# Deam0on/deepEMIA

Measured on AMD Instinct MI355X. Metric: EM tiles/s (2048x2048, R101-FPN), higher is better.
Workload: dtype f16x2

## Files before the change

### deepemia_amd/csrc/conv_p32.hip

```cpp
#include <utility>
#include "common.h"
#ifndef P32_ABLATE
#define P32_ABLATE 0
#endif

#ifndef P32_HEAD_DIRECT
#define P32_HEAD_DIRECT 1
#endif
#ifndef P32_SINGLE
#define P32_SINGLE 0
#endif
#ifndef P32_DEV_TILES
#define P32_DEV_TILES 0
#endif
#ifndef P32_ST_AUX
#define P32_ST_AUX 0
#endif
#ifndef P32_RES_AUX
#define P32_RES_AUX 0
#endif
#ifndef P32_A_NT
#define P32_A_NT 0
#endif
#ifndef P32_FRAG_PIPE
#define P32_FRAG_PIPE 0
#endif

namespace {

struct ConvQ {
    const void* in;
    const float* in_meta;
    const void* w;
    const float* scale;
    const float* bias;
    const void* res;
    const float* res_meta;
    void* out;
    float* out_meta;
    float wbound, bbound;
    int N, H, W, Cin, Ho, Wo, Cout, CoutPad, KH, KW, stride, pad;
    int act, res_mode, out_f32, out_ld;
    int M, HoWo, ntn, nwg, ksteps, taps;
    int kloop;
    unsigned in_bytes, w_bytes;
    unsigned out_bytes, res_bytes;
    const float* head_w;
    const float* head_b;
    float* head_out;
    int head_n, head_ld, head_act;
    int groups, group_rows, row0;
    int no_hk;
    int zero_low;
    int stagger_ticks;
    int resident;
};

typedef __attribute__((address_space(3))) void lds_void;

template <int OFF, int WAIT>
__device__ __forceinline__ void ds_read2_b128(f16x8& a, f16x8& b, unsigned addr_a, unsigned addr_b) {
    if constexpr (WAIT >= 0)
        asm volatile("ds_read_b128 %0, %2 offset:%4\n\tds_read_b128 %1, %3 offset:%4\n\ts_waitcnt lgkmcnt(%5)"
                     : "=&v"(a), "=&v"(b) : "v"(addr_a), "v"(addr_b), "n"(OFF), "n"(WAIT) : "memory");
    else
        asm volatile("ds_read_b128 %0, %2 offset:%4\n\tds_read_b128 %1, %3 offset:%4"
                     : "=&v"(a), "=&v"(b) : "v"(addr_a), "v"(addr_b), "n"(OFF) : "memory");
}

template <int... Is, class F>
__device__ __forceinline__ void static_for_impl(std::integer_sequence<int, Is...>, F&& f) { (f(std::integral_constant<int, Is>{}), ...); }
template <int N, class F>
__device__ __forceinline__ void static_for(F&& f) { static_for_impl(std::make_integer_sequence<int, N>{}, static_cast<F&&>(f)); }
typedef int i32x4 __attribute__((ext_vector_type(4)));

__device__ __forceinline__ void dma16(const i32x4 rsrc, unsigned lds_addr, unsigned voff, unsigned soff) {
    unsigned keep;
    asm volatile("s_mov_b32 %0, m0\n\ts_mov_b32 m0, %1\n\ts_nop 0\n\tbuffer_load_dwordx4 %2, %3, %4 offen lds\n\ts_mov_b32 m0, %0"
                 : "=&s"(keep) : "s"(lds_addr), "v"(voff), "s"(rsrc), "s"(soff) : "memory");
}
__device__ __forceinline__ void dma16_nt(const i32x4 rsrc, unsigned lds_addr, unsigned voff, unsigned soff) {
    unsigned keep;
    asm volatile("s_mov_b32 %0, m0\n\ts_mov_b32 m0, %1\n\ts_nop 0\n\tbuffer_load_dwordx4 %2, %3, %4 offen nt lds\n\ts_mov_b32 m0, %0"
                 : "=&s"(keep) : "s"(lds_addr), "v"(voff), "s"(rsrc), "s"(soff) : "memory");
}
__device__ __forceinline__ i32x4 make_rsrc(const void* base, unsigned bytes) {
    const unsigned long long a = reinterpret_cast<unsigned long long>(base);
    i32x4 r;
    r[0] = __builtin_amdgcn_readfirstlane((int)(unsigned)a);
    r[1] = __builtin_amdgcn_readfirstlane((int)((unsigned)(a >> 32) & 0xffffu));
    r[2] = __builtin_amdgcn_readfirstlane((int)bytes);
    r[3] = 0x00020000;
    return r;
}

__device__ __forceinline__ float apply_act_q(float v, int act) {
    if (act == DEMIA_ACT_RELU) return v > 0.f ? v : 0.f;
    if (act == DEMIA_ACT_SIGMOID) return 1.0f / (1.0f + expf(-v));
    return v;
}

__device__ __forceinline__ float plane_scale(float bound) {
    if (!(bound > 0.f) || !(bound < 3.0e38f)) return 1.f;
    int e = 14 - ilogbf(bound);
    e = e < -100 ? -100 : (e > 100 ? 100 : e);
    return ldexpf(1.f, e);
}

template <int TN, int EF>
__device__ __forceinline__ void write_acc32(const f32x16 (&row)[TN], float* e, int lane) {
#pragma unroll
    for (int j = 0; j < TN; ++j)
#pragma unroll
        for (int r = 0; r < 16; ++r)
            e[((r & 3) + 8 * (r >> 2) + 4 * (lane >> 5)) * EF + j * 32 + (lane & 31)] = row[j][r];
}
template <int TN, int EF>
__device__ __forceinline__ void write_acc16(const f32x4 (&r0)[2 * TN], const f32x4 (&r1)[2 * TN], float* e, int lane) {
#pragma unroll
    for (int j = 0; j < 2 * TN; ++j)
#pragma unroll
        for (int r = 0; r < 4; ++r) {
            e[(4 * (lane >> 4) + r) * EF + j * 16 + (lane & 15)] = r0[j][r];
            e[(16 + 4 * (lane >> 4) + r) * EF + j * 16 + (lane & 15)] = r1[j][r];
        }
}

__device__ __forceinline__ float uniform(float v) { return __int_as_float(__builtin_amdgcn_readfirstlane(__float_as_int(v))); }

struct GroupScales {
    int g0, b1, b2;
    float post0, post1, post2, resi0, resi1, resi2, sout0, sout1, sout2;
};

__device__ __forceinline__ void load_group_scale(const ConvQ& p, int gi, bool planes_out, float& post, float& resi, float& sout) {
    gi = min(gi, p.groups - 1);
    const float amax_in = p.in_meta[2 * gi], s_in = p.in_meta[2 * gi + 1];
    float amax_res = 0.f, s_res = 1.f;
    if (p.res_mode != DEMIA_RES_NONE) { amax_res = p.res_meta[2 * gi]; s_res = p.res_meta[2 * gi + 1]; }
    post = uniform(1.0f / s_in);
    resi = uniform(p.res_mode != DEMIA_RES_NONE ? 1.0f / s_res : 0.f);
    sout = uniform(planes_out ? plane_scale(amax_in * p.wbound + p.bbound + amax_res) : 1.f);
}

__device__ __forceinline__ GroupScales load_group_scales(const ConvQ& p, int m0, bool planes_out) {
    GroupScales gs;
    gs.g0 = (m0 + p.row0) / p.group_rows;
    gs.b1 = (gs.g0 + 1) * p.group_rows - p.row0;
    gs.b2 = gs.b1 + p.group_rows;
    load_group_scale(p, gs.g0, planes_out, gs.post0, gs.resi0, gs.sout0);
    load_group_scale(p, gs.g0 + 1, planes_out, gs.post1, gs.resi1, gs.sout1);
    load_group_scale(p, gs.g0 + 2, planes_out, gs.post2, gs.resi2, gs.sout2);
    return gs;
}

template <int WM, int WN, int TM, int TN, bool HEAD, typename WriteRow>
__device__ __forceinline__ void p32_epilogue(const ConvQ& p, const GroupScales& gs, char* smem, WriteRow&& write_tile_row, int wm, int wn, int m0, int n0) {
    constexpr int BN = WN * TN * 32;
    const int tid = threadIdx.x, lane = tid & 63;
    constexpr int EROW = BN * 4 + 16;
    constexpr int GPR = BN / 8, RSTEP = 512 / GPR, ITEMS = WM * 32 / RSTEP;
    static_assert(512 % GPR == 0 && (WM * 32) % RSTEP == 0, "epilogue split");
    constexpr int BM_ = WM * TM * 32;
    static_assert(!HEAD || BN == 256, "the fused head needs a 256-wide tile");
    const bool planes_out = !HEAD && !p.out_f32;
    const int g0 = __builtin_amdgcn_readfirstlane(gs.g0), b1 = __builtin_amdgcn_readfirstlane(gs.b1), b2 = __builtin_amdgcn_readfirstlane(gs.b2);
    const float post0 = uniform(gs.post0), post1 = uniform(gs.post1), post2 = uniform(gs.post2);
    const float resi0 = uniform(gs.resi0), resi1 = uniform(gs.resi1), resi2 = uniform(gs.resi2);
    const float sout0 = uniform(gs.sout0), sout1 = uniform(gs.sout1), sout2 = uniform(gs.sout2);
    if (planes_out && n0 == 0 && tid == 0) {
#pragma unroll
        for (int d = 0; d < 3; ++d) {
            const int first = d == 0 ? g0 * p.group_rows - p.row0 : (d == 1 ? b1 : b2);
            if (g0 + d < p.groups && first >= m0 && first < m0 + BM_ && first < p.M)
                p.out_meta[2 * (g0 + d) + 1] = d == 0 ? sout0 : (d == 1 ? sout1 : sout2);
        }
    }
    const int g = tid % GPR, r_first = tid / GPR;
    const int co = n0 + g * 8;
    float sc[8], bs[8];
#pragma unroll
    for (int q = 0; q < 8; ++q) {
        const bool ok = (co + q) < p.Cout;
        sc[q] = (p.scale && ok) ? p.scale[co + q] : 1.0f;
        bs[q] = (p.bias && ok) ? p.bias[co + q] : 0.0f;
    }
    float vmax3[3] = {0.f, 0.f, 0.f};
    constexpr int HMAX = 4;
    float hw[HMAX][8];
    constexpr bool head_on = HEAD;
    if (head_on) {
#pragma unroll
        for (int j = 0; j < HMAX; ++j)
#pragma unroll
            for (int q = 0; q < 8; ++q) hw[j][q] = j < p.head_n ? p.head_w[j * 256 + g * 8 + q] : 0.f;
    }
    const int tile_n_ = n0 / BN;
    const bool res_on = p.res_mode != DEMIA_RES_NONE, sigmoid_on = p.act == DEMIA_ACT_SIGMOID;
    const float act_lo = p.act == DEMIA_ACT_RELU ? 0.f : -INFINITY;
    const char* resb = reinterpret_cast<const char*>(p.res) + 128;
    char* outb = reinterpret_cast<char*>(p.out) + 128;
    const long cbytes = (long)p.Cout * 4;
    const int gofs = (co >> 5) * 128 + ((co & 31) >> 3) * 16;
    auto row_of = [&](int i, int k) { const int lr = r_first + k * RSTEP; return m0 + (lr >> 5) * (TM * 32) + i * 32 + (lr & 31); };
    auto res_pix = [&](int m) -> long {
        if (p.res_mode == DEMIA_RES_SAME) return m;
        const int n = m / p.HoWo;
        const int rem = m - n * p.HoWo;
// ... 194 lines not shown
    load_res(0);
#pragma unroll
    for (int i = 0; i < TM; ++i) {
        asm volatile("" ::: "memory");
        __builtin_amdgcn_wave_barrier();
        write_tile_row(i, reinterpret_cast<float*>(wsm));
        asm volatile("" ::: "memory");
        __builtin_amdgcn_wave_barrier();
        f16x8 ch[ITEMS], cl[ITEMS];
#pragma unroll
        for (int k = 0; k < ITEMS; ++k) {
            ch[k] = __builtin_bit_cast(f16x8, from_below(rh[k], rl[k]));
            cl[k] = __builtin_bit_cast(f16x8, from_above(rl[k], rh[k]));
        }
        if (i + 1 < TM) load_res(i + 1);
#pragma unroll
        for (int k = 0; k < ITEMS; ++k) {
            const int lr = r_first + k * RPI;
            const int m = row_of(i, k);
            const float4 x0 = *reinterpret_cast<const float4*>(wsm + lr * (LDW * 4) + (line * 4 + cj) * 32);
            const float4 x1 = *reinterpret_cast<const float4*>(wsm + lr * (LDW * 4) + (line * 4 + cj) * 32 + 16);
            typedef float f32x2 __attribute__((ext_vector_type(2)));
            f32x2 v2[4] = {{x0.x, x0.y}, {x0.z, x0.w}, {x1.x, x1.y}, {x1.z, x1.w}};
            const int gd = (m >= b1) + (m >= b2);
            const float post = gd == 0 ? post0 : (gd == 1 ? post1 : post2);
            const float res_inv = gd == 0 ? resi0 : (gd == 1 ? resi1 : resi2);
            const float s_out = gd == 0 ? sout0 : (gd == 1 ? sout1 : sout2);
            float v[8];
#pragma unroll
            for (int q = 0; q < 4; ++q) {
                const f32x2 scq = {sc[2 * q], sc[2 * q + 1]}, bsq = {bs[2 * q], bs[2 * q + 1]};
                const f32x2 t = (v2[q] * post) * scq + bsq;
                v[2 * q] = t.x;
                v[2 * q + 1] = t.y;
            }
#pragma unroll
            for (int q = 0; q < 8; ++q) {
                v[q] = fmaf((float)cl[k][q], res_inv, fmaf((float)ch[k][q], res_inv, v[q]));
                v[q] = fmaxf(v[q], act_lo);
            }
            if (sigmoid_on && !(P32_ABLATE & 256)) {
#pragma unroll
                for (int q = 0; q < 8; ++q) v[q] = 1.0f / (1.0f + expf(-v[q]));
            }
            f16x8 h, l;
            float vm = 0.f;
#pragma unroll
            for (int q = 0; q < 8; q += 2) {
                vm = fmaxf(vm, fmaxf(fabsf(v[q]), fabsf(v[q + 1])));
                const f32x2 y = f32x2{v[q], v[q + 1]} * s_out;
                h[q] = (_Float16)y.x;
                h[q + 1] = (_Float16)y.y;
                l[q] = (_Float16)fmaf(-(float)h[q], 1.0f, y.x);
                l[q + 1] = (_Float16)fmaf(-(float)h[q + 1], 1.0f, y.y);
            }
            if (single) l = f16x8{0, 0, 0, 0, 0, 0, 0, 0};
            vm = m < p.M ? vm : 0.f;
            vmax0 = fmaxf(vmax0, gd == 0 ? vm : 0.f);
            vmax1 = fmaxf(vmax1, gd == 1 ? vm : 0.f);
            vmax2 = fmaxf(vmax2, gd == 2 ? vm : 0.f);
            const u32x4 hu = __builtin_bit_cast(u32x4, h), lu = __builtin_bit_cast(u32x4, l);
            const u32x4 d0 = from_below(hu, lu);
            const u32x4 d1 = from_above(lu, hu);
            const unsigned off = (unsigned)(m - rs) * cbytes + lofs;
            if (P32_ABLATE & 64) {
                asm volatile("" :: "v"(d0), "v"(d1), "v"(off));
            } else {
                __builtin_amdgcn_raw_buffer_store_b128(d0, rs_out, off, 0, P32_ST_AUX);
                __builtin_amdgcn_raw_buffer_store_b128(d1, rs_out, off + cbytes, 0, P32_ST_AUX);
            }
            hook();
        }
    }
#pragma unroll
    for (int d = 0; d < 3; ++d) {
        if (d > 0 && (d == 1 ? b1 : b2) >= m0 + BM_) break;
        if (g0 + d >= p.groups) break;
        float vmax = d == 0 ? vmax0 : (d == 1 ? vmax1 : vmax2);
#pragma unroll
        for (int o = 32; o > 0; o >>= 1) vmax = fmaxf(vmax, __shfl_xor(vmax, o));
        float* slot = p.out_meta + 2 * (g0 + d);
        if (lane == 0 && vmax > *reinterpret_cast<volatile const float*>(slot))
            atomicMax(reinterpret_cast<unsigned int*>(slot), __float_as_uint(vmax));
    }
}

template <int WM, int WN, int TM, int TN, int HN>
__device__ __forceinline__ void p32_epilogue_head_direct(const ConvQ& p, const GroupScales& gs, char* smem, const f32x4 (&acc16)[2 * TM][2 * TN],
                                                         int wm, int wn, int m0, int n0) {
    constexpr int BM = WM * TM * 32, BN = WN * TN * 32;
    static_assert(BN == 256, "the fused head needs a 256-wide tile");
    const int tid = threadIdx.x, lane = tid & 63, c16 = lane & 15, rq = lane >> 4;
    const int b1 = __builtin_amdgcn_readfirstlane(gs.b1), b2 = __builtin_amdgcn_readfirstlane(gs.b2);
    const float post0 = uniform(gs.post0), post1 = uniform(gs.post1), post2 = uniform(gs.post2);
    float sc[2 * TN], bs[2 * TN], hw[HN][2 * TN];
#pragma unroll
    for (int jn = 0; jn < 2 * TN; ++jn) {
        const int cl = wn * TN * 32 + jn * 16 + c16;
        sc[jn] = p.scale ? p.scale[n0 + cl] : 1.0f;
        bs[jn] = p.bias ? p.bias[n0 + cl] : 0.0f;
#pragma unroll
        for (int j = 0; j < HN; ++j) hw[j][jn] = j < p.head_n ? p.head_w[j * 256 + cl] : 0.f;
    }
    const float act_lo = p.act == DEMIA_ACT_RELU ? 0.f : -INFINITY;
    float* part = reinterpret_cast<float*>(smem);
#pragma unroll
    for (int i = 0; i < 2 * TM; ++i) {
#pragma unroll
        for (int r = 0; r < 4; ++r) {
            const int row = wm * TM * 32 + i * 16 + rq * 4 + r;
            const int m = m0 + row;
            const int gd = (m >= b1) + (m >= b2);
            const float post = gd == 0 ? post0 : (gd == 1 ? post1 : post2);
            float a[HN];
#pragma unroll
            for (int j = 0; j < HN; ++j) a[j] = 0.f;
#pragma unroll
            for (int jn = 0; jn < 2 * TN; ++jn) {
                const float v = fmaxf((acc16[i][jn][r] * post) * sc[jn] + bs[jn], act_lo);
#pragma unroll
                for (int j = 0; j < HN; ++j) a[j] = fmaf(v, hw[j][jn], a[j]);
            }
#pragma unroll
            for (int j = 0; j < HN; ++j) {
                a[j] += __int_as_float(__builtin_amdgcn_update_dpp(0, __float_as_int(a[j]), 0x128, 0xf, 0xf, false));
                a[j] += __int_as_float(__builtin_amdgcn_update_dpp(0, __float_as_int(a[j]), 0x124, 0xf, 0xf, false));
                a[j] += __int_as_float(__builtin_amdgcn_update_dpp(0, __float_as_int(a[j]), 0x122, 0xf, 0xf, false));
                a[j] += __int_as_float(__builtin_amdgcn_update_dpp(0, __float_as_int(a[j]), 0x121, 0xf, 0xf, false));
            }
            if (c16 == 0) {
#pragma unroll
                for (int j = 0; j < HN; ++j) part[((long)wn * BM + row) * HN + j] = a[j];
            }
        }
    }
    __syncthreads();
    const int tile_n_ = n0 / BN;
    for (int o = tid; o < BM * HN; o += WM * WN * 64) {
        const int row = o / HN, j = o - row * HN;
        const int m = m0 + row;
        if (m >= p.M || j >= p.head_n) continue;
        float z = 0.f;
#pragma unroll
        for (int w = 0; w < WN; ++w) z += part[((long)w * BM + row) * HN + j];
        z += p.head_b[j];
        p.head_out[((long)m * p.ntn + tile_n_) * p.head_ld + j] =
            p.head_act == DEMIA_ACT_SIGMOID ? 1.0f / (1.0f + expf(-z)) : (p.head_act == DEMIA_ACT_RELU ? fmaxf(z, 0.f) : z);
    }
}


constexpr int EPI_GENERIC = 0, EPI_PLANES = 1, EPI_HEAD = 2;

template <int WM, int WN, int TM, int TN, bool M16 = true, int EPI = EPI_PLANES, int NST = 2, bool HK = false>
__global__ __launch_bounds__(WM * WN * 64, WM * WN == 8 ? 2 : 1) void conv_p32_kernel(const ConvQ p) {
    static_assert(NST == 2 || NST == 3, "two or three LDS stages");
    static_assert(!HK || (P32_SINGLE && M16 && NST == 2), "HK is a variant of the single-plane 16x16x32 kernel");
    static_assert(WM * WN == 8 || (WM * WN == 4 && EPI == EPI_PLANES), "eight waves, or four (planes epilogue only)");
    constexpr int NW = WM * WN;
    constexpr int BM = WM * TM * 32, BN = WN * TN * 32;
    constexpr int STAGE = (BM + BN) * 128;
    constexpr int NIA = BM / 8, NIB = BN / 8;

    extern __shared__ __attribute__((aligned(16))) char smem[];
    const int tid = threadIdx.x, lane = tid & 63;
    const int wave = __builtin_amdgcn_readfirstlane(tid >> 6);
    const int wm = wave / WN, wn = wave % WN;
    const int swz = xcd_remap(blockIdx.x, p.nwg);
    const int tile_n = swz % p.ntn, tile_m = swz / p.ntn;
    const int m0 = tile_m * BM, n0 = tile_n * BN;
#if P32_DEV_TILES
    if (p.stagger_ticks > 0) {
        const int b = blockIdx.x;
        const bool late = p.resident > 256 ? (b >= p.resident / 2 && b < p.resident) : (b < p.resident && ((b >> 3) & 1));
        if (late) {
            const unsigned long long t0 = __builtin_amdgcn_s_memrealtime();
            while (__builtin_amdgcn_s_memrealtime() - t0 < (unsigned long long)p.stagger_ticks) __builtin_amdgcn_s_sleep(32);
        }
    }
#endif

    const i32x4 rsrc_a = make_rsrc(p.in, p.in_bytes), rsrc_b = make_rsrc(p.w, p.w_bytes);
    const unsigned lds0 = (unsigned)(__SIZE_TYPE__)((lds_void*)smem);

    constexpr int QA = (NIA + NW - 1) / NW, QB = NIB / NW;
    constexpr bool A_EVEN = NIA % NW == 0;
    static_assert(NIB % NW == 0, "tile width is a multiple of 64");
    unsigned a_off[QA], a_msk[QA], b_off[QB];
#pragma unroll
    for (int q = 0; q < QA; ++q) {
        const int row = (wave + NW * q) * 8 + (lane >> 3);
        const int csw = (lane & 7) ^ ((row >> 1) & 7);
        const int m = m0 + row;
        const bool vm = m < p.M && row < BM;
        const int mm = vm ? m : 0;
        const int n = mm / p.HoWo;
        const int rem = mm - n * p.HoWo;
        const int ho = rem / p.Wo, wo = rem - ho * p.Wo;
        const int hi0 = ho * p.stride - p.pad, wi0 = wo * p.stride - p.pad;
        const long pix = ((long)n * p.H + hi0) * p.W + wi0;
        a_off[q] = (unsigned)(128 + pix * (long)(p.Cin * 4) + (HK ? (csw >> 2) * 128 + (csw & 3) * 16 : csw * 16));
        unsigned mk = 0;
        for (int t = 0, th = 0, tw = 0; t < p.taps; ++t) {
            if (vm && (unsigned)(hi0 + th) < (unsigned)p.H && (unsigned)(wi0 + tw) < (unsigned)p.W) mk |= 1u << t;
            if (++tw == p.KW) { tw = 0; ++th; }
        }
        a_msk[q] = mk;
    }
#pragma unroll
    for (int q = 0; q < QB; ++q) {
        const int row = (wave + NW * q) * 8 + (lane >> 3);
        const int csw = (lane & 7) ^ ((row >> 1) & 7);
        const int co = n0 + row;
        b_off[q] = (unsigned)(((co >> 6) * p.ksteps) * 8192 + (co & 63) * 128 + (HK ? (csw >> 2) * (p.taps * 8192) + (csw & 3) * 16 : csw * 16));
    }
    int tap = 0, kw = 0, tstep = 0;
    unsigned sdelta = 0, srow = 0, sgrp = 0;
    const bool a_nt = P32_A_NT && p.taps == 1 && p.ntn == 1;
    auto issue = [&](int st, int tp, unsigned sd, unsigned bd) {
        const unsigned sbase = __builtin_amdgcn_readfirstlane(lds0 + st * STAGE + wave * 1024);
        const bool first = bd < 2 * 8192u;
#pragma unroll
        for (int q = 0; q < QA; ++q) {
            if ((P32_ABLATE & 1) && !first) break;
            if (!A_EVEN && q == QA - 1 && wave + NW * q >= NIA) break;
            const bool ok = (a_msk[q] >> tp) & 1u;
            const unsigned vo = ok ? a_off[q] + sd : (a_off[q] & 0x70u);
            if (P32_A_NT && a_nt) dma16_nt(rsrc_a, sbase + q * (NW * 1024), vo, 0u);
            else dma16(rsrc_a, sbase + q * (NW * 1024), vo, 0u);
        }
#pragma unroll
        for (int q = 0; q < QB; ++q) {
            if ((P32_ABLATE & 2) && !first) break;
            dma16(rsrc_b, sbase + BM * 128 + q * (NW * 1024), b_off[q], bd);
        }
    };
    const unsigned pixb = (unsigned)(p.Cin * 4), rowb = (unsigned)(p.W * p.Cin * 4);
#define P32_ADVANCE()                                                                   \
    do {                                                                                \
        ++tstep;                                                                        \
        if (++tap == p.taps) { tap = 0; kw = 0; srow = 0; sgrp += HK ? 256u : 128u; sdelta = sgrp; if (HK) tstep += p.taps; } \
        else if (++kw == p.KW) { kw = 0; srow += rowb; sdelta = srow + sgrp; }          \
        else sdelta += pixb;                                                            \
    } while (0)

    const int fsw = (lane >> 1) & 7, hh = lane >> 5;
    int fa[4], fb[4];
#pragma unroll
    for (int c = 0; c < 4; ++c) {
        const int ch = (((c >> 1) * 4 + (c & 1) * 2 + hh) ^ fsw) * 16;
        fa[c] = (wm * TM * 32 + (lane & 31)) * 128 + ch;
        fb[c] = BM * 128 + (wn * TN * 32 + (lane & 31)) * 128 + ch;
    }

    f32x16 acc[M16 ? 1 : TM][M16 ? 1 : TN];
    f32x4 acc16[M16 ? 2 * TM : 1][M16 ? 2 * TN : 1];
#pragma unroll
    for (int i = 0; i < (M16 ? 1 : TM); ++i)
#pragma unroll
        for (int j = 0; j < (M16 ? 1 : TN); ++j)
#pragma unroll
            for (int r = 0; r < 16; ++r) acc[i][j][r] = 0.f;
#pragma unroll
    for (int i = 0; i < (M16 ? 2 * TM : 1); ++i)
#pragma unroll
        for (int j = 0; j < (M16 ? 2 * TN : 1); ++j)
#pragma unroll
            for (int r = 0; r < 4; ++r) acc16[i][j][r] = 0.f;
    int fa16[2], fb16[2];
#pragma unroll
    for (int pl = 0; pl < 2; ++pl) {
        const int ch = ((pl * 4 + (lane >> 4)) ^ (((lane & 15) >> 1) & 7)) * 16;
        fa16[pl] = (wm * TM * 32 + (lane & 15)) * 128 + ch;
        fb16[pl] = BM * 128 + (wn * TN * 32 + (lane & 15)) * 128 + ch;
    }

    constexpr bool BARRIER_IN_COMPUTE = (P32_FRAG_PIPE == 2) && M16 && NST == 2;
    auto compute1 = [&](int st) {
        const char* sb = smem + st * STAGE;
        if constexpr (M16) {
            f16x8 bh[2 * TN];
#pragma unroll
            for (int j = 0; j < 2 * TN; ++j) bh[j] = *reinterpret_cast<const f16x8*>(sb + fb16[0] + j * 2048);
#pragma unroll
            for (int i = 0; i < 2 * TM; ++i) {
                const f16x8 ah = *reinterpret_cast<const f16x8*>(sb + fa16[0] + i * 2048);
#pragma unroll
                for (int j = 0; j < 2 * TN; ++j) acc16[i][j] = __builtin_amdgcn_mfma_f32_16x16x32_f16(ah, bh[j], acc16[i][j], 0, 0, 0);
            }
        } else {
#pragma unroll
            for (int kk = 0; kk < 2; ++kk) {
                f16x8 bh[TN];
#pragma unroll
                for (int j = 0; j < TN; ++j) bh[j] = *reinterpret_cast<const f16x8*>(sb + fb[kk] + j * 4096);
#pragma unroll
                for (int i = 0; i < TM; ++i) {
                    const f16x8 ah = *reinterpret_cast<const f16x8*>(sb + fa[kk] + i * 4096);
#pragma unroll
                    for (int j = 0; j < TN; ++j) acc[i][j] = __builtin_amdgcn_mfma_f32_32x32x16_f16(ah, bh[j], acc[i][j], 0, 0, 0);
                }
            }
        }
        if (BARRIER_IN_COMPUTE) asm volatile("s_waitcnt vmcnt(0) lgkmcnt(0)\n\ts_barrier" ::: "memory");
    };
    auto compute_hk = [&](int st) {
        const char* sb = smem + st * STAGE;
        f16x8 b0[2 * TN], b1[2 * TN];
#pragma unroll
        for (int j = 0; j < 2 * TN; ++j) {
            b0[j] = *reinterpret_cast<const f16x8*>(sb + fb16[0] + j * 2048);
            b1[j] = *reinterpret_cast<const f16x8*>(sb + fb16[1] + j * 2048);
        }
#pragma unroll
        for (int i = 0; i < 2 * TM; ++i) {
            const f16x8 a0 = *reinterpret_cast<const f16x8*>(sb + fa16[0] + i * 2048);
            const f16x8 a1 = *reinterpret_cast<const f16x8*>(sb + fa16[1] + i * 2048);
#pragma unroll
            for (int j = 0; j < 2 * TN; ++j) {
                f32x4 c = acc16[i][j];
                c = __builtin_amdgcn_mfma_f32_16x16x32_f16(a0, b0[j], c, 0, 0, 0);
                c = __builtin_amdgcn_mfma_f32_16x16x32_f16(a1, b1[j], c, 0, 0, 0);
                acc16[i][j] = c;
            }
        }
    };
    auto compute = [&](int st) {
        if constexpr (HK) { compute_hk(st); return; }
        if constexpr (P32_SINGLE != 0) { compute1(st); return; }
        const char* sb = smem + st * STAGE;
        if constexpr (M16) {
            f16x8 bh[2 * TN], bl[2 * TN];
            f16x8 fake;
#pragma unroll
            for (int q = 0; q < 8; ++q) fake[q] = (_Float16)(float)(lane + q);
#if P32_FRAG_PIPE != 2
#pragma unroll
            for (int j = 0; j < 2 * TN; ++j) {
                bh[j] = (P32_ABLATE & 1024) ? fake : *reinterpret_cast<const f16x8*>(sb + fb16[0] + j * 2048);
                bl[j] = (P32_ABLATE & 1024) ? fake : *reinterpret_cast<const f16x8*>(sb + fb16[1] + j * 2048);
            }
#endif
#if P32_FRAG_PIPE == 2
            const unsigned la0 = (unsigned)(__SIZE_TYPE__)((lds_void*)(smem)) + st * STAGE + fa16[0];
            const unsigned la1 = la0 - fa16[0] + fa16[1];
            const unsigned lb0 = la0 - fa16[0] + fb16[0], lb1 = la0 - fa16[0] + fb16[1];
            f16x8 ahp[2], alp[2];
            ds_read2_b128<0, -1>(ahp[0], alp[0], la0, la1);
            static_for<2 * TN>([&](auto jc) {
                constexpr int j = decltype(jc)::value;
                ds_read2_b128<j * 2048, -1>(bh[j], bl[j], lb0, lb1);
            });
            static_for<2 * TM>([&](auto ic) {
                constexpr int i = decltype(ic)::value;
                const f16x8 ah = ahp[i & 1], al = alp[i & 1];
                if constexpr (i == 0) {
                    ds_read2_b128<2048, -1>(ahp[1], alp[1], la0, la1);
                    static_for<2 * TN>([&](auto jc) {
                        constexpr int j = decltype(jc)::value;
                        asm volatile("s_waitcnt lgkmcnt(%0)" ::"n"(2 * (2 * TN - 1 - j) + 2) : "memory");
                        __builtin_amdgcn_sched_barrier(0);
                        f32x4 c = acc16[0][j];
                        c = __builtin_amdgcn_mfma_f32_16x16x32_f16(ah, bl[j], c, 0, 0, 0);
                        c = __builtin_amdgcn_mfma_f32_16x16x32_f16(al, bh[j], c, 0, 0, 0);
                        c = __builtin_amdgcn_mfma_f32_16x16x32_f16(ah, bh[j], c, 0, 0, 0);
                        acc16[0][j] = c;
                        __builtin_amdgcn_sched_barrier(0);
                    });
                } else {
                    if constexpr (i + 1 < 2 * TM) {
                        ds_read2_b128<(i + 1) * 2048, 2>(ahp[(i + 1) & 1], alp[(i + 1) & 1], la0, la1);
                    } else if constexpr (BARRIER_IN_COMPUTE) {
                        asm volatile("s_waitcnt vmcnt(0) lgkmcnt(0)\n\ts_barrier" ::: "memory");
                    } else {
                        asm volatile("s_waitcnt lgkmcnt(0)" ::: "memory");
                    }
                    __builtin_amdgcn_sched_barrier(0);
#pragma unroll
                    for (int j = 0; j < 2 * TN; ++j) {
                        f32x4 c = acc16[i][j];
                        c = __builtin_amdgcn_mfma_f32_16x16x32_f16(ah, bl[j], c, 0, 0, 0);
                        c = __builtin_amdgcn_mfma_f32_16x16x32_f16(al, bh[j], c, 0, 0, 0);
                        c = __builtin_amdgcn_mfma_f32_16x16x32_f16(ah, bh[j], c, 0, 0, 0);
                        acc16[i][j] = c;
                    }
                    __builtin_amdgcn_sched_barrier(0);
                }
            });
            return;
#elif P32_FRAG_PIPE
            f16x8 ahp[2], alp[2];
            ahp[0] = *reinterpret_cast<const f16x8*>(sb + fa16[0]);
            alp[0] = *reinterpret_cast<const f16x8*>(sb + fa16[1]);
#pragma unroll
            for (int i = 0; i < 2 * TM; ++i) {
                if (i + 1 < 2 * TM) {
                    ahp[(i + 1) & 1] = *reinterpret_cast<const f16x8*>(sb + fa16[0] + (i + 1) * 2048);
                    alp[(i + 1) & 1] = *reinterpret_cast<const f16x8*>(sb + fa16[1] + (i + 1) * 2048);
                }
                const f16x8 ah = ahp[i & 1], al = alp[i & 1];
#pragma unroll
                for (int j = 0; j < 2 * TN; ++j) {
                    f32x4 c = acc16[i][j];
                    c = __builtin_amdgcn_mfma_f32_16x16x32_f16(ah, bl[j], c, 0, 0, 0);
                    c = __builtin_amdgcn_mfma_f32_16x16x32_f16(al, bh[j], c, 0, 0, 0);
                    c = __builtin_amdgcn_mfma_f32_16x16x32_f16(ah, bh[j], c, 0, 0, 0);
                    acc16[i][j] = c;
                }
                if (i + 1 < 2 * TM) __builtin_amdgcn_sched_group_barrier(0x100, 2, 0);
                __builtin_amdgcn_sched_group_barrier(0x008, 6 * TN, 0);
            }
            return;
#else
#pragma unroll
            for (int i = 0; i < 2 * TM; ++i) {
                const f16x8 ah = (P32_ABLATE & 1024) ? fake : *reinterpret_cast<const f16x8*>(sb + fa16[0] + i * 2048);
                const f16x8 al = (P32_ABLATE & 1024) ? fake : *reinterpret_cast<const f16x8*>(sb + fa16[1] + i * 2048);
#pragma unroll
                for (int j = 0; j < 2 * TN; ++j) {
                    f32x4 c = acc16[i][j];
                    if (P32_ABLATE & 4) {
                        asm volatile("" :: "v"(ah), "v"(al), "v"(bh[j]), "v"(bl[j]));
                        continue;
                    }
                    c = __builtin_amdgcn_mfma_f32_16x16x32_f16(ah, bl[j], c, 0, 0, 0);
                    c = __builtin_amdgcn_mfma_f32_16x16x32_f16(al, bh[j], c, 0, 0, 0);
                    c = __builtin_amdgcn_mfma_f32_16x16x32_f16(ah, bh[j], c, 0, 0, 0);
                    acc16[i][j] = c;
                }
            }
            return;
#endif
        }
#pragma unroll
        for (int kk = 0; kk < 2; ++kk) {
            f16x8 bh[TN], bl[TN];
#pragma unroll
            for (int j = 0; j < TN; ++j) {
                bh[j] = *reinterpret_cast<const f16x8*>(sb + fb[kk] + j * 4096);
                bl[j] = *reinterpret_cast<const f16x8*>(sb + fb[2 + kk] + j * 4096);
            }
#pragma unroll
            for (int i = 0; i < TM; ++i) {
                const f16x8 ah = *reinterpret_cast<const f16x8*>(sb + fa[kk] + i * 4096);
                const f16x8 al = *reinterpret_cast<const f16x8*>(sb + fa[2 + kk] + i * 4096);
#pragma unroll
                for (int j = 0; j < TN; ++j) {
                    f32x16 c = acc[i][j];
                    if (P32_ABLATE & 4) {
                        asm volatile("" :: "v"(ah), "v"(al), "v"(bh[j]), "v"(bl[j]));
                        continue;
                    }
                    c = __builtin_amdgcn_mfma_f32_32x32x16_f16(ah, bl[j], c, 0, 0, 0);
                    c = __builtin_amdgcn_mfma_f32_32x32x16_f16(al, bh[j], c, 0, 0, 0);
                    c = __builtin_amdgcn_mfma_f32_32x32x16_f16(ah, bh[j], c, 0, 0, 0);
                    acc[i][j] = c;
                }
            }
        }
    };

    constexpr int N_LAST = QB + QA, N_LAST_SHORT = QB + QA - 1;
    const bool short_wave = !A_EVEN && wave + NW * (QA - 1) >= NIA;
    auto wait_all_but_last_issue = [&]() {
        if (short_wave) asm volatile("s_waitcnt vmcnt(%0)" ::"n"(N_LAST_SHORT) : "memory");
        else asm volatile("s_waitcnt vmcnt(%0)" ::"n"(N_LAST) : "memory");
    };
    issue(0, tap, sdelta, 0u);
    P32_ADVANCE();
    bool two_ahead = false;
    if (NST == 3 && p.kloop > 1 && !(P32_ABLATE & 128)) {
        issue(1, tap, sdelta, (unsigned)tstep * 8192u);
        P32_ADVANCE();
        two_ahead = true;
    }
    constexpr bool HEAD = EPI == EPI_HEAD;
    const GroupScales gs = load_group_scales(p, m0, !HEAD && !p.out_f32);
    if (two_ahead) wait_all_but_last_issue();
    else asm volatile("s_waitcnt vmcnt(0)" ::: "memory");
    __builtin_amdgcn_s_barrier();
    int st = 0;
    for (int t = 0; t < ((P32_ABLATE & 128) ? 1 : p.kloop); ++t) {
        const int st_issue = NST == 2 ? (st ^ 1) : (st == 0 ? 2 : st - 1);
        const bool more = t + NST - 1 < p.kloop;
        if (more) {
            issue(st_issue, tap, sdelta, (unsigned)tstep * 8192u);
            P32_ADVANCE();
        }
        compute(st);
        if (NST == 3 && more) {
            wait_all_but_last_issue();
            asm volatile("s_waitcnt lgkmcnt(0)\n\ts_barrier" ::: "memory");
        } else if (!BARRIER_IN_COMPUTE) {
            asm volatile("s_waitcnt vmcnt(0) lgkmcnt(0)\n\ts_barrier" ::: "memory");
        }
        st = NST == 2 ? (st ^ 1) : (st == 2 ? 0 : st + 1);
    }
#undef P32_ADVANCE

    if constexpr ((P32_ABLATE & 2048) != 0 && M16) {
#pragma unroll
        for (int i = 0; i < 2 * TM; ++i)
#pragma unroll
            for (int j = 0; j < 2 * TN; ++j) asm volatile("" :: "v"(acc16[i][j]));
        return;
    }
    if constexpr (EPI == EPI_PLANES) {
        if constexpr (M16) {
            p32_epilogue_planes<WM, WN, TM, TN>(p, gs, smem, [&](int i, float* e) { write_acc16<TN, TN * 32 + 4>(acc16[2 * i], acc16[2 * i + 1], e, lane); }, wm, wn, m0, n0);
        } else {
            p32_epilogue_planes<WM, WN, TM, TN>(p, gs, smem, [&](int i, float* e) { write_acc32<TN, TN * 32 + 4>(acc[i], e, lane); }, wm, wn, m0, n0);
        }
    } else if constexpr (M16 && HEAD && P32_HEAD_DIRECT) {
        if (p.act != DEMIA_ACT_SIGMOID && p.head_n <= 2)
            p32_epilogue_head_direct<WM, WN, TM, TN, 2>(p, gs, smem, acc16, wm, wn, m0, n0);
        else
            p32_epilogue<WM, WN, TM, TN, HEAD>(p, gs, smem, [&](int i, float* e) { write_acc16<TN, BN + 4>(acc16[2 * i], acc16[2 * i + 1], e, lane); }, wm, wn, m0, n0);
    } else if constexpr (M16) {
        p32_epilogue<WM, WN, TM, TN, HEAD>(p, gs, smem, [&](int i, float* e) { write_acc16<TN, BN + 4>(acc16[2 * i], acc16[2 * i + 1], e, lane); }, wm, wn, m0, n0);
    } else {
        p32_epilogue<WM, WN, TM, TN, HEAD>(p, gs, smem, [&](int i, float* e) { write_acc32<TN, BN + 4>(acc[i], e, lane); }, wm, wn, m0, n0);
    }
}

#if P32_DEV_TILES
#include "conv_p32_dev.inc"
#endif

template <int WM, int WN, int TM, int TN, bool M16 = true, int EPI = EPI_PLANES, int NST = 2, bool HK = false>
int launch_q_(ConvQ p, hipStream_t st) {
    constexpr int BM = WM * TM * 32, BN = WN * TN * 32;
    constexpr int stages = NST * (BM + BN) * 128, image = EPI == EPI_PLANES ? WM * WN * 32 * (TN * 128 + 16) : WM * 32 * (BN * 4 + 16);
    static_assert(stages <= 160 * 1024, "LDS");
    constexpr int smem = stages > image ? stages : image;
    p.ntn = p.CoutPad / BN;
    p.nwg = p.ntn * cdiv(p.M, BM);
    p.resident = 256 * (160 * 1024 / smem >= 2 ? 2 : 1);
    p.kloop = HK ? p.ksteps / 2 : p.ksteps;
    auto k = conv_p32_kernel<WM, WN, TM, TN, M16, EPI, NST, HK>;
    static bool attr_done = false;
    if (!attr_done) {
        (void)hipFuncSetAttribute(reinterpret_cast<const void*>(k), hipFuncAttributeMaxDynamicSharedMemorySize, smem);
        attr_done = true;
    }
    hipLaunchKernelGGL(k, dim3(p.nwg), dim3(WM * WN * 64), smem, st, p);
    DEMIA_CHECK_LAUNCH("conv_p32_kernel");
    return DEMIA_OK;
}
template <int WM, int WN, int TM, int TN, bool M16 = true, int EPI = EPI_PLANES, int NST = 2>
int launch_q(ConvQ p, hipStream_t st) {
#if P32_SINGLE
    if constexpr (M16 && NST == 2) {
        if (p.Cin % 64 == 0 && !p.no_hk) return launch_q_<WM, WN, TM, TN, M16, EPI, NST, true>(p, st);
    }
#endif
    return launch_q_<WM, WN, TM, TN, M16, EPI, NST, false>(p, st);
}

struct TileCfg { int id, bm, bn; };
constexpr TileCfg kTiles[] = {{1, 256, 256}, {2, 128, 256}, {4, 192, 256}, {12, 160, 256}, {13, 224, 256}, {6, 256, 128}, {7, 128, 128}, {9, 256, 64}, {11, 128, 64}};

inline double predict_us(const TileCfg& c, long M, int cout_pad, int ksteps, bool residual) {
    const long tiles = (long)cdiv(M, c.bm) * (cout_pad / c.bn);
    const int smem = 2 * (c.bm + c.bn) * 128;
    const int occ = 160 * 1024 / smem >= 2 ? 2 : 1;
    const double area = (double)c.bm * c.bn / 65536.0;
    const double step = 2.0 * area * (1.0 + 0.2 * (1.0 - area));
    const double edge = 6.0 + 6.0 * area * (residual ? 1.5 : 1.0);
    if (occ == 1) return (double)((tiles + 255) / 256) * (ksteps * step + edge);
    return (double)((tiles + 511) / 512) * (2.0 * ksteps * step + 2.0 * 0.5 * edge);
}

inline int choose_tile(long M, int cout_pad, int ksteps, bool residual, bool need256 = false) {
#if P32_SINGLE
    if (cout_pad % 256 == 0 && (long)cdiv(M, 256) * (cout_pad / 256) >= 512) return 1;
#endif
    int best = 0;
    double best_t = 1e30;
    for (const TileCfg& c : kTiles) {
        if (cout_pad % c.bn || (need256 && c.bn != 256)) continue;
        const double t = predict_us(c, M, cout_pad, ksteps, residual);
        if (t < best_t) { best_t = t; best = c.id; }
    }
    return best;
}

}

#if P32_SINGLE
extern "C" int demia_conv2d_p32_single(const demia_conv_p32_desc* d, void* stream) {
#else
extern "C" int demia_conv2d_p32_single(const demia_conv_p32_desc* d, void* stream);
extern "C" int demia_conv2d_p32(const demia_conv_p32_desc* d, void* stream) {
    if (d && d->single) return demia_conv2d_p32_single(d, stream);
#endif
    DEMIA_REQUIRE(d && d->in && d->in_meta && d->w && (d->out || d->head_n > 0), "null pointer");
    DEMIA_REQUIRE(d->out_f32 || d->out_meta || d->head_n > 0, "P32 output needs out_meta");
    DEMIA_REQUIRE(d->Cin > 0 && d->Cin % 32 == 0, "Cin must be a multiple of 32");
    DEMIA_REQUIRE(d->CoutPad >= d->Cout && d->CoutPad % 64 == 0, "CoutPad must be a multiple of 64");
    DEMIA_REQUIRE(d->out_f32 || d->Cout % 32 == 0, "P32 output needs Cout % 32 == 0");
    DEMIA_REQUIRE(d->KH > 0 && d->KW > 0 && d->KH * d->KW <= 32 && d->stride > 0 && d->pad >= 0, "kernel geometry");
    DEMIA_REQUIRE(d->Ho == (d->H + 2 * d->pad - d->KH) / d->stride + 1, "Ho");
    DEMIA_REQUIRE(d->Wo == (d->W + 2 * d->pad - d->KW) / d->stride + 1, "Wo");
    DEMIA_REQUIRE(d->res_mode == DEMIA_RES_NONE || (d->residual && d->res_meta), "residual pointer");
    DEMIA_REQUIRE((long)d->N * d->Ho * d->Wo < (1L << 31), "M overflow");
    const long in_bytes = 128 + (long)d->N * d->H * d->W * d->Cin * 4;
    DEMIA_REQUIRE(in_bytes < (1L << 32), "input planes must stay below 4 GiB");
    const long w_bytes = (long)d->CoutPad * d->KH * d->KW * d->Cin * 4;
    DEMIA_REQUIRE(w_bytes < (1L << 31), "weight planes must stay below 2 GiB");
    ConvQ p;
    p.in = d->in; p.in_meta = d->in_meta; p.w = d->w; p.scale = d->scale; p.bias = d->bias;
    p.res = d->residual; p.res_meta = d->res_meta; p.out = d->out; p.out_meta = d->out_meta;
    p.wbound = d->wbound; p.bbound = d->bbound;
    p.N = d->N; p.H = d->H; p.W = d->W; p.Cin = d->Cin; p.Ho = d->Ho; p.Wo = d->Wo; p.Cout = d->Cout; p.CoutPad = d->CoutPad;
    p.KH = d->KH; p.KW = d->KW; p.stride = d->stride; p.pad = d->pad;
    p.act = d->act; p.res_mode = d->res_mode; p.out_f32 = d->out_f32;
    p.out_ld = d->out_ld > 0 ? d->out_ld : d->Cout;
    DEMIA_REQUIRE(p.out_ld >= d->Cout, "out_ld");
    p.M = d->N * d->Ho * d->Wo;
    p.HoWo = d->Ho * d->Wo;
    p.taps = d->KH * d->KW;
    p.ksteps = p.taps * (d->Cin / 32);
    p.in_bytes = (unsigned)in_bytes; p.w_bytes = (unsigned)w_bytes;
    p.ntn = p.nwg = 0;
    p.zero_low = d->single == 2;
    {
        static const char* env = getenv("DEMIA_P32_NO_HK");
        p.no_hk = (env && env[0] == '1') ? 1 : 0;
    }
    p.kloop = 0;
    p.resident = 256;
    p.groups = d->groups > 1 ? d->groups : 1;
    p.group_rows = p.groups > 1 ? d->group_rows : (1 << 29);
    p.row0 = p.groups > 1 ? d->row0 : 0;
    DEMIA_REQUIRE(p.groups == 1 || (d->group_rows >= 128 && d->row0 >= 0 && ((long)p.M + d->row0 + d->group_rows - 1) / d->group_rows <= p.groups),
                  "scale groups: group_rows >= 128 and the rows of this call must fall inside `groups` groups");
    p.head_w = d->head_w; p.head_b = d->head_b; p.head_out = d->head_out; p.head_n = d->head_n; p.head_ld = d->head_ld; p.head_act = d->head_act;
    if (d->head_n > 0) {
        DEMIA_REQUIRE(d->head_n <= 4 && d->head_w && d->head_b && d->head_out && d->head_ld >= d->head_n, "fused head: at most 4 rows, pointers, head_ld");
        DEMIA_REQUIRE(d->CoutPad % 256 == 0 && d->Cout == d->CoutPad && !d->out_f32, "fused head needs Cout % 256 == 0 and a planes layer");
    }
    p.stagger_ticks = 0;
#if P32_DEV_TILES
    {
        static const char* env = getenv("DEMIA_P32_STAGGER_US");
        p.stagger_ticks = env ? atoi(env) * 100 : 0;
    }
#endif
    if (p.M == 0) return DEMIA_OK;
    hipStream_t st = reinterpret_cast<hipStream_t>(stream);
    int tile = d->tile_hint ? d->tile_hint : choose_tile(p.M, d->CoutPad, p.ksteps, d->res_mode != DEMIA_RES_NONE, d->head_n > 0);
    const bool n256 = d->CoutPad % 256 == 0, n128 = d->CoutPad % 128 == 0;
    if (d->head_n > 0) {
        switch (tile) {
            case 1: return launch_q<2, 4, 4, 2, true, EPI_HEAD>(p, st);
            case 2: return launch_q<2, 4, 2, 2, true, EPI_HEAD>(p, st);
            default: return launch_q<1, 8, 6, 1, true, EPI_HEAD>(p, st);
        }
    }
    const int tile_bn = (tile == 9 || tile == 10 || tile == 11 || tile == 49) ? 64 : ((tile >= 6 && tile <= 8) || tile == 26 ? 128 : 256);
    const long out_bytes = 128 + (long)p.M * d->Cout * 4;
    long res_bytes = 0;
    if (d->res_mode == DEMIA_RES_SAME) res_bytes = out_bytes;
    if (d->res_mode == DEMIA_RES_UP2) res_bytes = 128 + (long)d->N * ((d->Ho + 1) / 2) * ((d->Wo + 1) / 2) * d->Cout * 4;
    const bool planes = !d->out_f32 && d->Cout % tile_bn == 0 && out_bytes < (1L << 32) - 512 && res_bytes < (1L << 32) - 512 &&
                        (long)(p.M + 256) * d->Cout * 4 + 256 < (1L << 32);
    p.out_bytes = (unsigned)out_bytes; p.res_bytes = (unsigned)res_bytes;
#if !P32_SINGLE && P32_DEV_TILES
    if (tile == 60) {
        DEMIA_REQUIRE(!d->out_f32 && n128 && d->Cout % 128 == 0 && d->KH == 1 && d->KW == 1 && d->stride == 1 && d->pad == 0 &&
                      d->res_mode != DEMIA_RES_UP2 && out_bytes < (1L << 32) - 512 && res_bytes < (1L << 32) - 512 &&
                      (long)(p.M + 256) * d->Cout * 4 + 256 < (1L << 32),
                      "tile 60 (ping-pong) takes 1x1 stride-1 planes layers with Cout % 128 == 0, no nearest-2x residual, buffers below 4 GiB");
        return launch_pp1x1(p, st);
    }
#endif
    if (!planes) {
        if (tile != 7 && tile != 9 && tile != 10 && tile != 11 && tile != 21 && tile != 22 && tile != 26) tile = n128 ? 7 : 11;
        switch (tile) {
            case 7: DEMIA_REQUIRE(n128, "tile needs CoutPad % 128 == 0"); return launch_q<4, 2, 1, 2, true, EPI_GENERIC>(p, st);
            case 9: return launch_q<8, 1, 1, 2, true, EPI_GENERIC>(p, st);
            case 10: return launch_q<4, 2, 2, 1, true, EPI_GENERIC>(p, st);
            case 11: return launch_q<4, 2, 1, 1, true, EPI_GENERIC>(p, st);
            default: break;
        }
    }
    switch (tile) {
        case 1: DEMIA_REQUIRE(n256, "tile needs CoutPad % 256 == 0"); return launch_q<2, 4, 4, 2>(p, st);
        case 2: DEMIA_REQUIRE(n256, "tile needs CoutPad % 256 == 0"); return launch_q<2, 4, 2, 2>(p, st);
        case 4: DEMIA_REQUIRE(n256, "tile needs CoutPad % 256 == 0"); return launch_q<1, 8, 6, 1>(p, st);
        case 6: DEMIA_REQUIRE(n128, "tile needs CoutPad % 128 == 0"); return launch_q<4, 2, 2, 2>(p, st);
        case 7: DEMIA_REQUIRE(n128, "tile needs CoutPad % 128 == 0"); return launch_q<4, 2, 1, 2>(p, st);
        case 9: return launch_q<8, 1, 1, 2>(p, st);
        case 11: return launch_q<4, 2, 1, 1>(p, st);
        case 12: DEMIA_REQUIRE(n256, "tile needs CoutPad % 256 == 0"); return launch_q<1, 8, 5, 1>(p, st);
        case 13: DEMIA_REQUIRE(n256, "tile needs CoutPad % 256 == 0"); return launch_q<1, 8, 7, 1>(p, st);
#if P32_DEV_TILES
        case 3: DEMIA_REQUIRE(n256, "tile needs CoutPad % 256 == 0"); return launch_q<1, 8, 8, 1>(p, st);
        case 5: DEMIA_REQUIRE(n256, "tile needs CoutPad % 256 == 0"); return launch_q<1, 8, 4, 1>(p, st);
        case 8: DEMIA_REQUIRE(n128, "tile needs CoutPad % 128 == 0"); return launch_q<2, 4, 2, 1>(p, st);
        case 10: return launch_q<4, 2, 2, 1>(p, st);
        case 14: DEMIA_REQUIRE(n256, "tile needs CoutPad % 256 == 0"); return launch_q<2, 4, 3, 2>(p, st);
        case 42: DEMIA_REQUIRE(n256, "tile needs CoutPad % 256 == 0"); return launch_q<2, 4, 2, 2, true, EPI_PLANES, 3>(p, st);
        case 52: DEMIA_REQUIRE(n256, "tile needs CoutPad % 256 == 0"); return launch_q<1, 8, 5, 1, true, EPI_PLANES, 3>(p, st);
        case 49: return launch_q<8, 1, 1, 2, true, EPI_PLANES, 3>(p, st);
        case 31: DEMIA_REQUIRE(n256, "tile needs CoutPad % 256 == 0"); return launch_q<2, 4, 4, 2, false>(p, st);
        case 34: DEMIA_REQUIRE(n256, "tile needs CoutPad % 256 == 0"); return launch_q<1, 8, 6, 1, false>(p, st);
        case 21: DEMIA_REQUIRE(n256, "tile needs CoutPad % 256 == 0"); return launch_pp<4, 2>(p, st);
        case 22: DEMIA_REQUIRE(n256, "tile needs CoutPad % 256 == 0"); return launch_pp<2, 2>(p, st);
        case 26: DEMIA_REQUIRE(n128, "tile needs CoutPad % 128 == 0"); return launch_pp<4, 1>(p, st);
#endif
        default: DEMIA_REQUIRE(false, "tile_hint");
    }
    return DEMIA_EINVAL;
}
```

Before: 718.4.

## Add strip-mode 3x3 conv loading one padded row strip per kh, reused across kw taps

```diff
diff --git a/deepemia_amd/csrc/conv_p32.hip b/deepemia_amd/csrc/conv_p32.hip
--- a/deepemia_amd/csrc/conv_p32.hip
+++ b/deepemia_amd/csrc/conv_p32.hip
@@ -1,5 +1,6 @@
 #include <utility>
 #include "common.h"
+#include "conv_p32_strip.h"
 #ifndef P32_ABLATE
 #define P32_ABLATE 0
 #endif
@@ -54,6 +55,7 @@
     int zero_low;
     int stagger_ticks;
     int resident;
+    int strip_ok;
 };
 
 typedef __attribute__((address_space(3))) void lds_void;
@@ -554,9 +556,10 @@
 
 constexpr int EPI_GENERIC = 0, EPI_PLANES = 1, EPI_HEAD = 2;
 
-template <int WM, int WN, int TM, int TN, bool M16 = true, int EPI = EPI_PLANES, int NST = 2, bool HK = false>
+template <int WM, int WN, int TM, int TN, bool M16 = true, int EPI = EPI_PLANES, int NST = 2, bool HK = false, bool STRIP = false>
 __global__ __launch_bounds__(WM * WN * 64, WM * WN == 8 ? 2 : 1) void conv_p32_kernel(const ConvQ p) {
     static_assert(NST == 2 || NST == 3, "two or three LDS stages");
+    static_assert(!STRIP || (!P32_SINGLE && M16 && NST == 2 && !HK && EPI == EPI_PLANES && WM * WN == 8), "strip mode: two-plane 16x16x32 kernel, two stages, planes epilogue");
     static_assert(!HK || (P32_SINGLE && M16 && NST == 2), "HK is a variant of the single-plane 16x16x32 kernel");
     static_assert(WM * WN == 8 || (WM * WN == 4 && EPI == EPI_PLANES), "eight waves, or four (planes epilogue only)");
     constexpr int NW = WM * WN;
@@ -862,41 +865,143 @@
         }
     };
 
-    constexpr int N_LAST = QB + QA, N_LAST_SHORT = QB + QA - 1;
-    const bool short_wave = !A_EVEN && wave + NW * (QA - 1) >= NIA;
-    auto wait_all_but_last_issue = [&]() {
-        if (short_wave) asm volatile("s_waitcnt vmcnt(%0)" ::"n"(N_LAST_SHORT) : "memory");
-        else asm volatile("s_waitcnt vmcnt(%0)" ::"n"(N_LAST) : "memory");
-    };
-    issue(0, tap, sdelta, 0u);
-    P32_ADVANCE();
-    bool two_ahead = false;
-    if (NST == 3 && p.kloop > 1 && !(P32_ABLATE & 128)) {
-        issue(1, tap, sdelta, (unsigned)tstep * 8192u);
+    constexpr bool HEAD = EPI == EPI_HEAD;
+    GroupScales gs;
+    if constexpr (STRIP) {
+        namespace sp = p32strip;
+        constexpr int CAP = sp::cap_lines(BM), CAPB = CAP * 128, NPS = CAP / 8, QS = (NPS + NW - 1) / NW;
+        constexpr int BRING = 2 * CAPB, BSTAGE = BN * 128;
+        static_assert(CAP % 16 == 0, "the swizzle key (line >> 1) & 7 must not change with the slot");
+        (void)a_off; (void)a_msk; (void)fa16; (void)fb16; (void)issue; (void)compute; (void)srow; (void)sgrp; (void)kw; (void)tap; (void)sdelta; (void)pixb;
+        const int first = __builtin_amdgcn_readfirstlane(sp::tile_first(m0, p.W));
+        const int npt = __builtin_amdgcn_readfirstlane((sp::lines_needed(m0, BM, p.W) + 7) >> 3);
+        unsigned s_off[QS], s_val = 0;
+#pragma unroll
+        for (int q = 0; q < QS; ++q) {
+            const int line = (wave + NW * q) * 8 + (lane >> 3);
+            const unsigned cb = (unsigned)sp::swizzle(line, lane & 7) * 16u;
+            const sp::Source src = sp::source(first + line, p.W, p.H, p.M);
+            s_off[q] = src.valid ? 128u + (unsigned)src.pix * (unsigned)(p.Cin * 4) + cb : cb;
+            s_val |= src.valid << (3 * q);
+        }
+        unsigned fx[2 * TM], fbs[2];
+#pragma unroll
+        for (int i = 0; i < 2 * TM; ++i) fx[i] = (unsigned)sp::line_of(m0 + wm * TM * 32 + i * 16 + (lane & 15), 0, first, p.W) * 128u;
+#pragma unroll
+        for (int pl = 0; pl < 2; ++pl)
+            fbs[pl] = (unsigned)(BRING + (wn * TN * 32 + (lane & 15)) * 128 + ((pl * 4 + (lane >> 4)) ^ (((lane & 15) >> 1) & 7)) * 16);
+        unsigned c4 = (unsigned)(lane >> 4) * 16u;
+        auto frag_at = [](unsigned x0, unsigned sofs, unsigned c4_, unsigned& hi, unsigned& lo) {
+            const unsigned m70 = __builtin_amdgcn_readfirstlane(0x70);
+            asm volatile("v_add_u32 %0, %3, %2\n\tv_lshrrev_b32 %1, 4, %0\n\tv_xor_b32 %1, %1, %4\n\tv_and_or_b32 %0, %1, %5, %0\n\tv_xor_b32 %1, 64, %0"
+                         : "=&v"(hi), "=&v"(lo) : "v"(x0), "s"(sofs), "v"(c4_), "s"(m70));
+        };
+        auto issue_strip = [&](unsigned slot_base, auto sub_c, unsigned sd, int kh) {
+            constexpr int SUB = decltype(sub_c)::value;
+            static_for<QS>([&](auto qc) {
+                constexpr int q = decltype(qc)::value;
+                if constexpr (SUB == 3 || q % 3 == SUB) {
+                    if ((P32_ABLATE & 1) && SUB != 3) return;
+                    const int piece = wave + NW * q;
+                    if (piece < npt) {
+                        const bool ok = (s_val >> (3 * q + kh)) & 1u;
+                        const unsigned vo = ok ? s_off[q] + sd : (s_off[q] & 0x70u);
+                        dma16(rsrc_a, __builtin_amdgcn_readfirstlane(lds0 + slot_base + piece * 1024), vo, 0u);
+                    }
+                }
+            });
+        };
+        auto issue_b = [&](unsigned bst_base, unsigned bd) {
+            const unsigned sbase = __builtin_amdgcn_readfirstlane(lds0 + BRING + bst_base + wave * 1024);
+#pragma unroll
+            for (int q = 0; q < QB; ++q) dma16(rsrc_b, sbase + q * (NW * 1024), b_off[q], bd);
+        };
+        auto compute_strip = [&](unsigned sofs, unsigned bst_base) {
+            const char* sb = smem + bst_base;
+            f16x8 bh[2 * TN], bl[2 * TN];
+#pragma unroll
+            for (int j = 0; j < 2 * TN; ++j) {
+                bh[j] = *reinterpret_cast<const f16x8*>(sb + fbs[0] + j * 2048);
+                bl[j] = *reinterpret_cast<const f16x8*>(sb + fbs[1] + j * 2048);
+            }
+#pragma unroll
+            for (int i = 0; i < 2 * TM; ++i) {
+                unsigned ah_at, al_at;
+                frag_at(fx[i], sofs, c4, ah_at, al_at);
+                const f16x8 ah = *reinterpret_cast<const f16x8*>(smem + ah_at);
+                const f16x8 al = *reinterpret_cast<const f16x8*>(smem + al_at);
+#pragma unroll
+                for (int j = 0; j < 2 * TN; ++j) {
+                    f32x4 c = acc16[i][j];
+                    if (P32_ABLATE & 4) {
+                        asm volatile("" :: "v"(ah), "v"(al), "v"(bh[j]), "v"(bl[j]));
+                        continue;
+                    }
+                    c = __builtin_amdgcn_mfma_f32_16x16x32_f16(ah, bl[j], c, 0, 0, 0);
+                    c = __builtin_amdgcn_mfma_f32_16x16x32_f16(al, bh[j], c, 0, 0, 0);
+                    c = __builtin_amdgcn_mfma_f32_16x16x32_f16(ah, bh[j], c, 0, 0, 0);
+                    acc16[i][j] = c;
+                }
+            }
+        };
+        const int nstrips = (P32_ABLATE & 128) ? 1 : p.ksteps / 3;
+        int nkh = 1;
+        unsigned ngrp = 0;
+        issue_strip(0u, std::integral_constant<int, 3>{}, 0u - rowb, 0);
+        issue_b(0u, 0u);
+        gs = load_group_scales(p, m0, !p.out_f32);
+        asm volatile("s_waitcnt vmcnt(0)" ::: "memory");
+        __builtin_amdgcn_s_barrier();
+        for (int s = 0; s < nstrips; ++s) {
+            const unsigned slot_base = (unsigned)(s & 1) * CAPB;
+            const bool more = s + 1 < nstrips;
+            const unsigned sd = ngrp + (unsigned)nkh * rowb - rowb;
+            static_for<3>([&](auto kw_c) {
+                constexpr int KW = decltype(kw_c)::value;
+                const unsigned bst_base = (unsigned)((s + KW) & 1) * BSTAGE;
+                if (more) issue_strip(slot_base ^ CAPB, kw_c, sd, nkh);
+                if (KW < 2 || more) issue_b(bst_base ^ BSTAGE, (unsigned)(3 * s + KW + 1) * 8192u);
+                compute_strip(slot_base + KW * 128, bst_base);
+                asm volatile("s_waitcnt vmcnt(0) lgkmcnt(0)\n\ts_barrier" ::: "memory");
+            });
+            if (++nkh == 3) { nkh = 0; ngrp += 128u; }
+        }
+    } else {
+        constexpr int N_LAST = QB + QA, N_LAST_SHORT = QB + QA - 1;
+        const bool short_wave = !A_EVEN && wave + NW * (QA - 1) >= NIA;
+        auto wait_all_but_last_issue = [&]() {
+            if (short_wave) asm volatile("s_waitcnt vmcnt(%0)" ::"n"(N_LAST_SHORT) : "memory");
+            else asm volatile("s_waitcnt vmcnt(%0)" ::"n"(N_LAST) : "memory");
+        };
+        issue(0, tap, sdelta, 0u);
         P32_ADVANCE();
-        two_ahead = true;
-    }
-    constexpr bool HEAD = EPI == EPI_HEAD;
-    const GroupScales gs = load_group_scales(p, m0, !HEAD && !p.out_f32);
-    if (two_ahead) wait_all_but_last_issue();
-    else asm volatile("s_waitcnt vmcnt(0)" ::: "memory");
-    __builtin_amdgcn_s_barrier();
-    int st = 0;
-    for (int t = 0; t < ((P32_ABLATE & 128) ? 1 : p.kloop); ++t) {
-        const int st_issue = NST == 2 ? (st ^ 1) : (st == 0 ? 2 : st - 1);
-        const bool more = t + NST - 1 < p.kloop;
-        if (more) {
-            issue(st_issue, tap, sdelta, (unsigned)tstep * 8192u);
+        bool two_ahead = false;
+        if (NST == 3 && p.kloop > 1 && !(P32_ABLATE & 128)) {
+            issue(1, tap, sdelta, (unsigned)tstep * 8192u);
             P32_ADVANCE();
-        }
-        compute(st);
-        if (NST == 3 && more) {
-            wait_all_but_last_issue();
-            asm volatile("s_waitcnt lgkmcnt(0)\n\ts_barrier" ::: "memory");
-        } else if (!BARRIER_IN_COMPUTE) {
-            asm volatile("s_waitcnt vmcnt(0) lgkmcnt(0)\n\ts_barrier" ::: "memory");
-        }
-        st = NST == 2 ? (st ^ 1) : (st == 2 ? 0 : st + 1);
+            two_ahead = true;
+        }
+        gs = load_group_scales(p, m0, !HEAD && !p.out_f32);
+        if (two_ahead) wait_all_but_last_issue();
+        else asm volatile("s_waitcnt vmcnt(0)" ::: "memory");
+        __builtin_amdgcn_s_barrier();
+        int st = 0;
+        for (int t = 0; t < ((P32_ABLATE & 128) ? 1 : p.kloop); ++t) {
+            const int st_issue = NST == 2 ? (st ^ 1) : (st == 0 ? 2 : st - 1);
+            const bool more = t + NST - 1 < p.kloop;
+            if (more) {
+                issue(st_issue, tap, sdelta, (unsigned)tstep * 8192u);
+                P32_ADVANCE();
+            }
+            compute(st);
+            if (NST == 3 && more) {
+                wait_all_but_last_issue();
+                asm volatile("s_waitcnt lgkmcnt(0)\n\ts_barrier" ::: "memory");
+            } else if (!BARRIER_IN_COMPUTE) {
+                asm volatile("s_waitcnt vmcnt(0) lgkmcnt(0)\n\ts_barrier" ::: "memory");
+            }
+            st = NST == 2 ? (st ^ 1) : (st == 2 ? 0 : st + 1);
+        }
     }
 #undef P32_ADVANCE
 
@@ -929,17 +1034,17 @@
 #include "conv_p32_dev.inc"
 #endif
 
-template <int WM, int WN, int TM, int TN, bool M16 = true, int EPI = EPI_PLANES, int NST = 2, bool HK = false>
+template <int WM, int WN, int TM, int TN, bool M16 = true, int EPI = EPI_PLANES, int NST = 2, bool HK = false, bool STRIP = false>
 int launch_q_(ConvQ p, hipStream_t st) {
     constexpr int BM = WM * TM * 32, BN = WN * TN * 32;
-    constexpr int stages = NST * (BM + BN) * 128, image = EPI == EPI_PLANES ? WM * WN * 32 * (TN * 128 + 16) : WM * 32 * (BN * 4 + 16);
+    constexpr int stages = STRIP ? 2 * (p32strip::cap_lines(BM) + BN) * 128 : NST * (BM + BN) * 128, image = EPI == EPI_PLANES ? WM * WN * 32 * (TN * 128 + 16) : WM * 32 * (BN * 4 + 16);
     static_assert(stages <= 160 * 1024, "LDS");
     constexpr int smem = stages > image ? stages : image;
     p.ntn = p.CoutPad / BN;
     p.nwg = p.ntn * cdiv(p.M, BM);
     p.resident = 256 * (160 * 1024 / smem >= 2 ? 2 : 1);
     p.kloop = HK ? p.ksteps / 2 : p.ksteps;
-    auto k = conv_p32_kernel<WM, WN, TM, TN, M16, EPI, NST, HK>;
+    auto k = conv_p32_kernel<WM, WN, TM, TN, M16, EPI, NST, HK, STRIP>;
     static bool attr_done = false;
     if (!attr_done) {
         (void)hipFuncSetAttribute(reinterpret_cast<const void*>(k), hipFuncAttributeMaxDynamicSharedMemorySize, smem);
@@ -949,11 +1054,16 @@
     DEMIA_CHECK_LAUNCH("conv_p32_kernel");
     return DEMIA_OK;
 }
+constexpr bool strip_tile(int bm, int bn) { return (bm == 256 && bn == 128) || (bm == 128 && bn == 256) || (bm == 128 && bn == 64); }
 template <int WM, int WN, int TM, int TN, bool M16 = true, int EPI = EPI_PLANES, int NST = 2>
 int launch_q(ConvQ p, hipStream_t st) {
 #if P32_SINGLE
     if constexpr (M16 && NST == 2) {
         if (p.Cin % 64 == 0 && !p.no_hk) return launch_q_<WM, WN, TM, TN, M16, EPI, NST, true>(p, st);
+    }
+#else
+    if constexpr (M16 && NST == 2 && EPI == EPI_PLANES && strip_tile(WM * TM * 32, WN * TN * 32)) {
+        if (p.strip_ok && p32strip::admits(WM * TM * 32, p.W)) return launch_q_<WM, WN, TM, TN, M16, EPI, NST, false, true>(p, st);
     }
 #endif
     return launch_q_<WM, WN, TM, TN, M16, EPI, NST, false>(p, st);
@@ -1032,6 +1142,7 @@
     }
     p.kloop = 0;
     p.resident = 256;
+    p.strip_ok = d->KH == 3 && d->KW == 3 && d->stride == 1 && d->pad == 1 && !(d->tile_hint & 0x100);
     p.groups = d->groups > 1 ? d->groups : 1;
     p.group_rows = p.groups > 1 ? d->group_rows : (1 << 29);
     p.row0 = p.groups > 1 ? d->row0 : 0;
@@ -1051,7 +1162,7 @@
 #endif
     if (p.M == 0) return DEMIA_OK;
     hipStream_t st = reinterpret_cast<hipStream_t>(stream);
-    int tile = d->tile_hint ? d->tile_hint : choose_tile(p.M, d->CoutPad, p.ksteps, d->res_mode != DEMIA_RES_NONE, d->head_n > 0);
+    int tile = (d->tile_hint & 0xff) ? (d->tile_hint & 0xff) : choose_tile(p.M, d->CoutPad, p.ksteps, d->res_mode != DEMIA_RES_NONE, d->head_n > 0);
     const bool n256 = d->CoutPad % 256 == 0, n128 = d->CoutPad % 128 == 0;
     if (d->head_n > 0) {
         switch (tile) {
diff --git a/deepemia_amd/csrc/conv_p32_strip.h b/deepemia_amd/csrc/conv_p32_strip.h
--- /dev/null
+++ b/deepemia_amd/csrc/conv_p32_strip.h
@@ -0,0 +1,39 @@
+#pragma once
+
+#if defined(__HIPCC__)
+#define P32_STRIP_FN __host__ __device__ inline
+#else
+#define P32_STRIP_FN inline
+#endif
+
+namespace p32strip {
+
+constexpr int kSlackLines = 40;
+constexpr int kMinW = 8;
+
+P32_STRIP_FN constexpr int cap_lines(int bm) { return (bm + kSlackLines + 15) / 16 * 16; }
+
+P32_STRIP_FN int padded(int m, int W) { return m + m / W + 1; }
+P32_STRIP_FN int tile_first(int m0, int W) { return padded(m0, W) - 1; }
+P32_STRIP_FN int lines_needed(int m0, int bm, int W) { return padded(m0 + bm - 1, W) + 1 - tile_first(m0, W) + 1; }
+
+P32_STRIP_FN constexpr bool admits(int bm, int W) { return W >= kMinW && bm + 2 + (bm - 2) / W + 1 <= cap_lines(bm); }
+
+P32_STRIP_FN int line_of(int m, int kw, int first, int W) { return padded(m, W) + kw - 1 - first; }
+
+P32_STRIP_FN int swizzle(int line, int chunk) { return chunk ^ ((line >> 1) & 7); }
+
+struct Source { int pix; unsigned valid; };
+P32_STRIP_FN Source source(int q, int W, int H, int M) {
+    Source s = {0, 0u};
+    const int R = q / (W + 1), c = q - R * (W + 1);
+    if (c == 0) return s;
+    const int m = R * W + c - 1;
+    if (m >= M) return s;
+    const int ho = R % H;
+    s.pix = m;
+    s.valid = (ho > 0 ? 1u : 0u) | 2u | (ho + 1 < H ? 4u : 0u);
+    return s;
+}
+
+}
```

Result: no change. 723.7, median of 6 (+0.7%).
